# JunyiPeng00/wespeaker_hubert

Hardware: AMD Instinct MI355X
Metric: embeddings/sec on 5s 16kHz utts (higher is better)
Workload: dtype f32 (bf16x3 split MFMA, fp32 accumulate)

## Files before the change

### wespeaker_hubert_amd/csrc/conv_gemm.hip

```cpp
#include "gemm_common.h"

namespace wsp {

namespace {

constexpr int BK = 32;
constexpr int LDK = BK + 4;

template <int WM, int WN, int TM, int TN, int AMODE, bool UNI>
__global__ __launch_bounds__(256, 2) void conv_gemm_f32(const ConvGemmArgs p) {
  constexpr int BM = WM * TM * 32;
  constexpr int BN = WN * TN * 32;
  constexpr int AR = BM / 32;
  constexpr int BR = BN / 32;
  static_assert(WM * WN == 4, "4 waves");

  extern __shared__ __attribute__((aligned(16))) float smem[];
  float* As = smem;
  float* Bs = smem + 2 * BM * LDK;

  const int tid = threadIdx.x;
  const int lane = tid & 63;
  const int wave = tid >> 6;
  const int ntiles = p.N / BN;
// ... 79 lines not shown
}

template <int WM, int WN, int TM, int TN, int AMODE, bool UNI>
void launch_k(const ConvGemmArgs& p, hipStream_t s) {
  constexpr int BM = WM * TM * 32, BN = WN * TN * 32;
  const int nwg = ((p.M + BM - 1) / BM) * (p.N / BN);
  const size_t lds = (size_t)2 * (BM + BN) * LDK * sizeof(float);
  hipLaunchKernelGGL((conv_gemm_f32<WM, WN, TM, TN, AMODE, UNI>), dim3(nwg), dim3(256), lds, s, p);
  WSP_HIP(hipGetLastError());
}

template <int WM, int WN, int TM, int TN>
void launch_tile(const ConvGemmArgs& p, hipStream_t s) {
  const bool uni = uniform_ktiles(p);
  if (p.amode == kAAdd) {
    if (uni) launch_k<WM, WN, TM, TN, kAAdd, true>(p, s);
    else launch_k<WM, WN, TM, TN, kAAdd, false>(p, s);
  } else {
    if (uni) launch_k<WM, WN, TM, TN, kACat, true>(p, s);
    else launch_k<WM, WN, TM, TN, kACat, false>(p, s);
  }
}

}

int conv_gemm_tile_for(int N) { return (N % 128 == 0) ? 0 : 1; }

void launch_conv_gemm(const ConvGemmArgs& args, hipStream_t s) {
  const ConvGemmArgs p = normalized(args);
  check_conv_args(p, "conv_gemm");
  WSP_CHECK(!p.colsum, "conv_gemm: column sums are a bf16x3-kernel epilogue");
  WSP_CHECK(!p.conv2d && p.N % 64 == 0, "conv_gemm (f32): 1-D convs with N % 64 == 0 only");
  WSP_CHECK(!p.gcols || p.gcols % 64 == 0, "conv_gemm (f32): grouped columns must be a multiple of 64");
  WSP_CHECK(!p.sc2d && !p.lnmode, "conv_gemm (f32): conv3 + shortcut and the LayerNorm fold run on tile family 7");
  if (conv_gemm_tile_for(p.N) == 0 && !p.gcols)
    launch_tile<2, 2, 2, 2>(p, s);
  else
    launch_tile<4, 1, 1, 2>(p, s);
}

}
```

### wespeaker_hubert_amd/csrc/conv_gemm_x3.hip

```cpp
#include "conv_gemm_x3_impl.h"

namespace wsp {

int conv_gemm_x3_block_rows(const ConvGemmArgs& p, int variant) {
  if (p.N % 64 != 0 || (p.gcols && p.gcols % 64 != 0)) return 128;
  if (p.gcols || p.N % 128 != 0) return 128;
  return variant == 3 ? 128 : 256;
}

namespace {
__global__ __launch_bounds__(256) void colsum_mean_kernel(const double* __restrict__ part, int bm, int T, int N,
                                                          float* __restrict__ out, int ldo) {
  const int b = blockIdx.y;
  const int n = blockIdx.x * 256 + threadIdx.x;
  if (n >= N) return;
  const long r0 = (long)b * T, r1 = r0 + T;
  double v = 0.0;
  for (long mt = r0 / bm; mt * bm < r1; ++mt) {
    const int slot = (mt * bm) / T == b ? 0 : 1;
    v += part[((size_t)mt * 2 + slot) * N + n];
  }
  out[(long)b * ldo + n] = (float)(v / (double)T);
}
}

void launch_colsum_mean(const double* part, int block_rows, int T, int B, int N, float* out, int ldo,
                        hipStream_t s) {
  WSP_CHECK(block_rows > 0 && T >= block_rows && B > 0 && N > 0, "colsum_mean: bad shape");
  hipLaunchKernelGGL(colsum_mean_kernel, dim3((N + 255) / 256, B), dim3(256), 0, s, part, block_rows, T, N, out,
                     ldo);
  WSP_HIP(hipGetLastError());
}

void launch_conv_gemm_x3(const ConvGemmArgs& args, const void* whi, const void* wlo, int variant,
                         hipStream_t s) {
  const ConvGemmArgs p = normalized(args);
  check_conv_args(p, "conv_gemm_x3");
  if (p.colsum) {
    const int bm = conv_gemm_x3_block_rows(p, variant);
    WSP_CHECK(!p.seg && !p.row_bias && !p.conv2d && p.T >= bm,
              "conv_gemm_x3: column sums need a uniform batch with T >= block rows and no row bias");
  }
  WSP_CHECK(p.Kp % 64 == 0, "conv_gemm_x3: packed K must be a multiple of 64");
  WSP_CHECK(variant >= 3 && variant <= 7, "conv_gemm_x3: tile family must be 3, 4, 5, 6 or 7");
  const __bf16* h = static_cast<const __bf16*>(whi);
  const __bf16* l = static_cast<const __bf16*>(wlo);
  x3::TileFn f;
  WSP_CHECK(!p.lnmode || (variant == 7 && x3::g256_supported(p)),
            "conv_gemm_x3: the LayerNorm fold runs on tile family 7 only");
  WSP_CHECK(!p.sc2d || (variant == 7 && x3::g256_supported(p)),
            "conv_gemm_x3: conv3 + shortcut runs on tile family 7 only (N % 256 == 0, 16-B aligned operands)");
  if (variant == 7 && x3::g256_supported(p)) {
    x3::t_g256(p, h, l, s);
    return;
  }
  if (variant == 7) variant = 6;
  if (p.N % 64 != 0 || (p.gcols && p.gcols % 64 != 0)) {
    f = x3::t_4x1_1x1;
  } else if (p.gcols) {
    f = variant >= 5 ? x3::t_8x1_1x2_sw : x3::t_4x1_1x2;
  } else if (p.N % 128 != 0) {
    f = x3::t_4x1_1x2;
  } else if (variant == 3) {
    f = x3::t_2x2_2x2_sw;
  } else if (variant == 4) {
    f = x3::t_4x2_2x2_sw;
  } else if (p.N % 256 == 0) {
    f = variant == 6 ? x3::t_4x2_2x4_mf16 : x3::t_4x2_2x4_sw1;
  } else {
    f = x3::t_4x2_2x2_sw;
  }
  f(p, h, l, s);
}

}
```

### wespeaker_hubert_amd/csrc/conv_gemm_x3_impl.h

```cpp
#pragma once

#include <type_traits>

#include "gemm_common.h"

namespace wsp {

namespace {

typedef __bf16 bf16x8 __attribute__((ext_vector_type(8)));
typedef __bf16 bf16x4 __attribute__((ext_vector_type(4)));

constexpr int BK = 32;

template <bool SWZ, int MF = 32>
struct Lds {
  static constexpr int ROWB = SWZ ? 64 : 80;
  static constexpr int SKEW = SWZ ? 0 : 64;
  __device__ __forceinline__ static int off(int row, int byte) {
    static_assert(MF == 32 || SWZ, "16x16 fragments need the swizzled rows");
    if constexpr (SWZ && MF == 16)
      return row * 64 + ((((byte >> 4) ^ (0x1320 >> (4 * ((row >> 2) & 3)))) & 3) << 4) + (byte & 15);
    else if constexpr (SWZ) return row * 64 + ((((byte >> 4) ^ (row >> 2)) & 3) << 4) + (byte & 15);
    else return row * 80 + byte;
// ... 269 lines not shown
  if (MF == 32 && p.amode == kAAdd) {
    if constexpr (MF == 32) {
      if (uni)
        launch_x3_k<WM, WN, TM, TN, kAAdd, true, 0, false, SWZ, NSET, MF>(p, whi, wlo, s);
      else
        launch_x3_k<WM, WN, TM, TN, kAAdd, false, 0, false, SWZ, NSET, MF>(p, whi, wlo, s);
    }
  } else if (!uni) {
    launch_x3_k<WM, WN, TM, TN, kACat, false, 0, false, SWZ, NSET, MF>(p, whi, wlo, s);
  } else if (p.role == 1) {
    launch_x3_k<WM, WN, TM, TN, kACat, true, 1, false, SWZ, NSET, MF>(p, whi, wlo, s);
  } else if constexpr (NSET == 2 && TM * TN <= 4) {
    if (p.res && p.role == 2)
      launch_x3_k<WM, WN, TM, TN, kACat, true, 2, false, SWZ, NSET>(p, whi, wlo, s);
    else
      launch_x3_k<WM, WN, TM, TN, kACat, true, 0, false, SWZ, NSET>(p, whi, wlo, s);
  } else {
    launch_x3_k<WM, WN, TM, TN, kACat, true, 0, false, SWZ, NSET, MF>(p, whi, wlo, s);
  }
}

}

namespace x3 {
using TileFn = void (*)(const ConvGemmArgs&, const __bf16*, const __bf16*, hipStream_t);
void t_4x1_1x1(const ConvGemmArgs&, const __bf16*, const __bf16*, hipStream_t);
void t_4x1_1x2(const ConvGemmArgs&, const __bf16*, const __bf16*, hipStream_t);
void t_8x1_1x2_sw(const ConvGemmArgs&, const __bf16*, const __bf16*, hipStream_t);
void t_2x2_2x2_sw(const ConvGemmArgs&, const __bf16*, const __bf16*, hipStream_t);
void t_4x2_2x2_sw(const ConvGemmArgs&, const __bf16*, const __bf16*, hipStream_t);
void t_4x2_2x4_sw1(const ConvGemmArgs&, const __bf16*, const __bf16*, hipStream_t);
void t_4x2_2x4_mf16(const ConvGemmArgs&, const __bf16*, const __bf16*, hipStream_t);
bool g256_supported(const ConvGemmArgs&);
void t_g256(const ConvGemmArgs&, const __bf16*, const __bf16*, hipStream_t);
}

}
```

### wespeaker_hubert_amd/csrc/conv_gemm_x3_t6.hip

```cpp
#include "conv_gemm_x3_impl.h"

namespace wsp {
namespace {

typedef __attribute__((address_space(3))) void lds_void;
constexpr int kGA = 256 * 128, kGW = 256 * 64, kGStage = kGA + 2 * kGW;

__device__ __forceinline__ int g_aslot(int r, int c) { return r * 128 + ((c ^ ((r >> 1) & 5)) << 4); }

__device__ __forceinline__ void g_dma(__amdgpu_buffer_rsrc_t r, unsigned char* lds, int voff) {
  __builtin_amdgcn_raw_ptr_buffer_load_lds(r, (lds_void*)lds, 16, voff, 0, 0, 0);
}

constexpr int kGEpiLd = 132;
constexpr int kGEpiBytes = 8 * 32 * kGEpiLd * 4;
typedef unsigned u32x4 __attribute__((ext_vector_type(4)));

constexpr int kLnMaxParts = 8;
__device__ __forceinline__ void g_ln_row(const ConvGemmArgs& p, int row, float& mu, float& rstd) {
  const float* s = p.ln_in + (size_t)row * p.ln_parts * 2;
  float m = s[0], m2 = s[1];
#pragma unroll
  for (int k = 1; k < kLnMaxParts; ++k) {
    if (k < p.ln_parts) {
// ... 188 lines not shown
      v0 += __shfl_xor(v0, 32);
      double v1 = c1 + __shfl_xor(c1, 16);
      v1 += __shfl_xor(v1, 32);
      rs[4 * pp + jj][0] = v0;
      rs[4 * pp + jj][1] = v1;
      __builtin_amdgcn_sched_barrier(0);
    }
    asm volatile("s_waitcnt lgkmcnt(0)" ::: "memory");
  }
  __syncthreads();
  constexpr int BN = 256;
  double* red = reinterpret_cast<double*>(smem);
  if (lane < 16) {
#pragma unroll
    for (int j = 0; j < 8; ++j)
#pragma unroll
      for (int u = 0; u < 2; ++u) red[(wm * 2 + u) * BN + (wn * 8 + j) * 16 + lane] = rs[j][u];
  }
  __syncthreads();
  const int tid = threadIdx.x;
  if (tid < 2 * BN) {
    const int u = tid / BN, c = tid - u * BN;
    double v = 0.0;
#pragma unroll
    for (int w = 0; w < 4; ++w) v += red[(w * 2 + u) * BN + c];
    p.colsum[((size_t)(m0 / 256) * 2 + u) * p.N + n0 + c] = v;
  }
}

template <int AM, bool CSK, int LNM = 0, int XP = 0>
__global__ __launch_bounds__(512, 1) void conv_gemm_g(const ConvGemmArgs p, const __bf16* __restrict__ whi,
                                                      const __bf16* __restrict__ wlo) {
  using L = Lds<true, 16>;
  constexpr bool DENSE = AM == 1 || AM == 3;
  extern __shared__ __attribute__((aligned(16))) unsigned char smem[];
  const int tid = threadIdx.x;
  const int lane = tid & 63;
  const int wave = tid >> 6;
  const int ntiles = p.N / 256;
  const int mtiles = (p.M + 255) / 256;
  const int wg = xcd_remap(blockIdx.x, ntiles * mtiles);
  const int mt = wg / ntiles;
  const int nt = wg - mt * ntiles;
  const int m0 = mt * 256;
  const int n0 = nt * 256;

  const int ac0 = 4 * ((lane & 7) ^ ((lane >> 4) & 1)), ac1 = ac0 ^ 16;
  int a_r[4], a_t[DENSE ? 1 : 4], a_l[DENSE ? 1 : 4], a_s[AM == 3 ? 4 : 1];
#pragma unroll
  for (int i = 0; i < 4; ++i) {
    const int m = m0 + (4 * wave + i) * 8 + (lane >> 3);
    if constexpr (DENSE) {
      a_r[i] = m < p.M ? m : -1;
      if constexpr (AM == 3) {
        const int fto = p.Fo * p.To;
        const int b = m / fto, fo = (m - b * fto) / p.To, to = m - b * fto - fo * p.To;
        a_s[i] = m < p.M ? (b * p.Fi + fo * p.stride) * p.Ti + to * p.stride : -1;
      }
    } else if (p.seg) {
      const int mm = m < p.M ? m : p.M - 1;
      const int b = seg_of(p.seg, p.nseg, mm);
      const int t = (mm - p.seg[b]) * p.stride;
      const int* is = p.iseg ? p.iseg : p.seg;
      a_r[i] = is[b] + t;
      a_t[i] = (m < p.M) ? t : -0x40000000;
      a_l[i] = is[b + 1] - is[b];
    } else {
// ... 42 lines not shown
        const int offk = tap * p.dil - p.pad;
        const int tt = a_t[i] + offk;
        const bool ok = k < p.K && tt >= 0 && tt < a_l[i];
        g_dma(ra, st + (4 * wave + i) * 1024, ok ? ((a_r[i] + offk) * ld + k - tap * p.cin) * 4 : kOOB);
      } else {
        const int tt = a_t[i] + off;
        const bool ok = tt >= 0 && tt < a_l[i];
        g_dma(ra, st + (4 * wave + i) * 1024, ok ? ((a_r[i] + off) * ld + cl + (i & 1 ? ac1 : ac0)) * 4 : kOOB);
      }
    }
#pragma unroll
    for (int i = 0; i < 2; ++i) {
      if (!(part & 2)) break;
      const int o = woff[i] + kt * 64;
      g_dma(rwh, st + kGA + (2 * wave + i) * 1024, o);
      g_dma(rwl, st + kGA + kGW + (2 * wave + i) * 1024, o);
    }
    if (!(part & 2)) return;
    ct += 32;
    if (ct >= p.cin) {
      ct -= p.cin;
      ++jt;
    }
  };

  const int wm = wave >> 1, wn = wave & 1;
  const int r16 = lane & 15, qk = lane >> 4;
  f32x4 acc[4][8];
#pragma unroll
  for (int i = 0; i < 4; ++i)
#pragma unroll
    for (int j = 0; j < 8; ++j) acc[i][j] = f32x4{0.f, 0.f, 0.f, 0.f};
  bf16x8 ah[2], al[2], bh[4], bl[4];
  auto rdA = [&](const unsigned char* st, int ih) {
#pragma unroll
    for (int i = 0; i < 2; ++i) {
      const int r = wm * 64 + (ih * 2 + i) * 16 + r16;
      const f32x4 x0 = *reinterpret_cast<const f32x4*>(st + g_aslot(r, 2 * qk));
      const f32x4 x1 = *reinterpret_cast<const f32x4*>(st + g_aslot(r, 2 * qk + 1));
      if constexpr (XP == 1 || XP == 4) {
        ah[i] = __builtin_bit_cast(bf16x8, x0);
        al[i] = __builtin_bit_cast(bf16x8, x1);
        continue;
      }
#pragma unroll
      for (int e = 0; e < 4; ++e) {
        const __bf16 h0 = (__bf16)x0[e], h1 = (__bf16)x1[e];
        ah[i][e] = h0;
        ah[i][4 + e] = h1;
        al[i][e] = (__bf16)(x0[e] - (float)h0);
        al[i][4 + e] = (__bf16)(x1[e] - (float)h1);
      }
    }
  };
  auto rdB = [&](const unsigned char* st, int jh) {
#pragma unroll
    for (int j = 0; j < 4; ++j) {
      const int o = L::off(wn * 128 + (jh * 4 + j) * 16 + r16, qk * 16);
      bh[j] = *reinterpret_cast<const bf16x8*>(st + kGA + o);
      bl[j] = *reinterpret_cast<const bf16x8*>(st + kGA + kGW + o);
    }
  };
  auto mm = [&](int ih, int jh) {
#pragma unroll
    for (int i = 0; i < 2; ++i)
#pragma unroll
      for (int j = 0; j < 4; ++j) {
        f32x4& c = acc[ih * 2 + i][jh * 4 + j];
        c = __builtin_amdgcn_mfma_f32_16x16x32_bf16(al[i], bh[j], c, 0, 0, 0);
        c = __builtin_amdgcn_mfma_f32_16x16x32_bf16(ah[i], bl[j], c, 0, 0, 0);
        c = __builtin_amdgcn_mfma_f32_16x16x32_bf16(ah[i], bh[j], c, 0, 0, 0);
      }
  };

  float lmu = 0.f, lrs = 1.f;
  if constexpr ((LNM & 6) != 0) g_ln_row(p, min(m0 + wm * 64 + lane, p.M - 1), lmu, lrs);
  dma(0, 0);
  dma(1, 1);
  asm volatile("s_waitcnt vmcnt(8)" ::: "memory");
  __builtin_amdgcn_s_barrier();
  for (int kt = 0; kt < nk; ++kt) {
    const int buf = kt & 1;
    const unsigned char* st = smem + buf * kGStage;
    if constexpr (XP == 2) {
      rdA(st, 0);
      rdB(st, 0);
      mm(0, 0);
      __builtin_amdgcn_sched_barrier(0);
      if (kt >= 1 && kt + 1 < nk) dma(kt + 1, buf ^ 1, 1);
      __builtin_amdgcn_sched_barrier(0);
      rdB(st, 1);
      mm(0, 1);
      __builtin_amdgcn_sched_barrier(0);
      if (kt >= 1 && kt + 1 < nk) dma(kt + 1, buf ^ 1, 2);
      __builtin_amdgcn_sched_barrier(0);
      rdA(st, 1);
      mm(1, 1);
      rdB(st, 0);
      mm(1, 0);
      asm volatile("s_waitcnt vmcnt(0) lgkmcnt(0)" ::: "memory");
      __builtin_amdgcn_s_barrier();
      __builtin_amdgcn_sched_barrier(0);
      continue;
    }
    rdA(st, 0);
    rdB(st, 0);
    mm(0, 0);
    rdB(st, 1);
    mm(0, 1);
    rdA(st, 1);
    mm(1, 1);
    rdB(st, 0);
    mm(1, 0);
    if constexpr (XP >= 3) {
      asm volatile("s_waitcnt lgkmcnt(0)" ::: "memory");
      continue;
    }
    asm volatile("s_waitcnt vmcnt(0) lgkmcnt(0)" ::: "memory");
    __builtin_amdgcn_s_barrier();
    __builtin_amdgcn_sched_barrier(0);
    if (kt + 2 < nk) dma(kt + 2, buf);
  }
#define WSP_GEPI(RB, RES)                                                                                   \
  switch (p.act) {                                                                                         \
    case kActRelu: g_epilogue_rows<kActRelu, RB, RES>(p, acc, m0, n0, wm, wn, wave, lane, smem); break;    \
    case kActTanh: g_epilogue_rows<kActTanh, RB, RES>(p, acc, m0, n0, wm, wn, wave, lane, smem); break;    \
    case kActGelu: g_epilogue_rows<kActGelu, RB, RES>(p, acc, m0, n0, wm, wn, wave, lane, smem); break;    \
    default: g_epilogue_rows<kActNone, RB, RES>(p, acc, m0, n0, wm, wn, wave, lane, smem); break;          \
  }
  if constexpr (LNM != 0) {
    if constexpr ((LNM & 5) != 0)
      g_epilogue_rows<kActNone, false, true, LNM>(p, acc, m0, n0, wm, wn, wave, lane, smem, lmu, lrs);
    else if (p.act == kActGelu)
      g_epilogue_rows<kActGelu, false, false, LNM>(p, acc, m0, n0, wm, wn, wave, lane, smem, lmu, lrs);
    else
      g_epilogue_rows<kActNone, false, false, LNM>(p, acc, m0, n0, wm, wn, wave, lane, smem, lmu, lrs);
  } else if constexpr (CSK) {
    switch (p.act) {
      case kActRelu: g_epilogue_cs<kActRelu>(p, acc, m0, n0, wm, wn, wave, lane, smem); break;
      case kActTanh: g_epilogue_cs<kActTanh>(p, acc, m0, n0, wm, wn, wave, lane, smem); break;
      case kActGelu: g_epilogue_cs<kActGelu>(p, acc, m0, n0, wm, wn, wave, lane, smem); break;
      default: g_epilogue_cs<kActNone>(p, acc, m0, n0, wm, wn, wave, lane, smem); break;
    }
  } else if (p.res) {
    WSP_GEPI(false, true)
  } else if (p.row_bias) {
    WSP_GEPI(true, false)
  } else {
    WSP_GEPI(false, false)
  }
#undef WSP_GEPI
}

#ifdef WSP_G7_XP
constexpr int kBStages = 4;
// ... 160 lines not shown
    default: g_epilogue_rows<kActNone, RB, RES>(p, acc, m0, n0, wm, wn, wave, lane, smem); break;          \
  }
  if constexpr (CSK) {
    switch (p.act) {
      case kActRelu: g_epilogue_cs<kActRelu>(p, acc, m0, n0, wm, wn, wave, lane, smem); break;
      case kActTanh: g_epilogue_cs<kActTanh>(p, acc, m0, n0, wm, wn, wave, lane, smem); break;
      case kActGelu: g_epilogue_cs<kActGelu>(p, acc, m0, n0, wm, wn, wave, lane, smem); break;
      default: g_epilogue_cs<kActNone>(p, acc, m0, n0, wm, wn, wave, lane, smem); break;
    }
  } else if (p.res) {
    WSP_GBEPI(false, true)
  } else if (p.row_bias) {
    WSP_GBEPI(true, false)
  } else {
    WSP_GBEPI(false, false)
  }
#undef WSP_GBEPI
}
#endif

}

namespace x3 {

bool g256_supported(const ConvGemmArgs& p) {
  auto a16 = [](const void* q) { return (reinterpret_cast<uintptr_t>(q) & 15) == 0; };
  const bool aligned = a16(p.out) && p.ldo % 4 == 0 && a16(p.bias) && a16(p.scale) && a16(p.shift) &&
                       a16(p.row_bias) && a16(p.res) && (!p.res || p.ldres % 4 == 0);
  return aligned && p.N % 256 == 0 && !p.conv2d && !p.gcols && p.amode == kACat &&
         (uniform_ktiles(p) || (p.cseg[1] >= p.cin && !p.colsum)) &&
         (!p.sc2d || (uniform_ktiles(p) && !p.colsum && !p.lnmode && !p.row_bias));
}

void t_g256(const ConvGemmArgs& p, const __bf16* h, const __bf16* l, hipStream_t s) {
  const int nwg = ((p.M + 255) / 256) * (p.N / 256);
  constexpr int lds0 = 2 * kGStage > kGEpiBytes ? 2 * kGStage : kGEpiBytes;
  constexpr int lds = lds0 > kGCsBytes ? lds0 : kGCsBytes;
  const bool dense = p.taps == 1 && p.pad == 0 && p.stride == 1 && !p.iseg && (p.seg || p.Ti == p.T);
  const int am = !uniform_ktiles(p) ? 2 : dense ? 1 : 0;
  if (p.sc2d) {
    hipLaunchKernelGGL((conv_gemm_g<3, false>), dim3(nwg), dim3(512), lds, s, p, h, l);
    WSP_HIP(hipGetLastError());
    return;
  }
  if (p.lnmode) {
    WSP_CHECK(am == 1 && !p.colsum && !p.row_bias && !p.scale && p.N % 128 == 0 &&
                  ((p.lnmode & 1) == 0 || (p.ln_out && p.res && p.act == kActNone)) &&
                  ((p.lnmode & 6) == 0 || (p.ln_in && p.ln_parts >= 1 && p.ln_parts <= kLnMaxParts)) && ((p.lnmode & 2) == 0 || (p.ln_cs && !p.res)) &&
                  (p.lnmode != 2 || p.act == kActNone || p.act == kActGelu) &&
                  ((p.lnmode & 4) == 0 || (p.ln_g && p.ln_b && p.res && p.act == kActNone)),
              "conv_gemm_x3: LayerNorm fold needs a dense 1x1 GEMM and its operands (fold: no activation or GELU)");
    switch (p.lnmode) {
      case 1: hipLaunchKernelGGL((conv_gemm_g<1, false, 1>), dim3(nwg), dim3(512), lds, s, p, h, l); break;
      case 2: hipLaunchKernelGGL((conv_gemm_g<1, false, 2>), dim3(nwg), dim3(512), lds, s, p, h, l); break;
      case 4: hipLaunchKernelGGL((conv_gemm_g<1, false, 4>), dim3(nwg), dim3(512), lds, s, p, h, l); break;
      case 5: hipLaunchKernelGGL((conv_gemm_g<1, false, 5>), dim3(nwg), dim3(512), lds, s, p, h, l); break;
      default: WSP_CHECK(false, "conv_gemm_x3: lnmode must be 1, 2, 4 or 5");
    }
    WSP_HIP(hipGetLastError());
    return;
  }
  if (p.colsum && am == 1)
    hipLaunchKernelGGL((conv_gemm_g<1, true>), dim3(nwg), dim3(512), lds, s, p, h, l);
  else if (p.colsum && am == 0)
    hipLaunchKernelGGL((conv_gemm_g<0, true>), dim3(nwg), dim3(512), lds, s, p, h, l);
  else if (am == 1)
    hipLaunchKernelGGL((conv_gemm_g<1, false>), dim3(nwg), dim3(512), lds, s, p, h, l);
  else if (am == 0)
    hipLaunchKernelGGL((conv_gemm_g<0, false>), dim3(nwg), dim3(512), lds, s, p, h, l);
  else
    hipLaunchKernelGGL((conv_gemm_g<2, false>), dim3(nwg), dim3(512), lds, s, p, h, l);
  WSP_HIP(hipGetLastError());
// ... 53 lines not shown
```

### wespeaker_hubert_amd/csrc/ecapa_model.cpp

```cpp
#include "model_impl.h"

namespace wsp {

void Model::Impl::build_ecapa_params() {
  const int64_t C = this->C, w = C / 8;
  add("layer1.conv.weight", {C, feat_dim, 5});
  add("layer1.conv.bias", {C});
  add_bn("layer1.bn", C);
  for (int li = 2; li <= 4; ++li) {
    const std::string p = "layer" + std::to_string(li) + ".se_res2block";
    add(p + ".0.conv.weight", {C, C, 1});
    add(p + ".0.conv.bias", {C});
    add_bn(p + ".0.bn", C);
    for (int i = 0; i < 7; ++i) {
      add(p + ".1.convs." + std::to_string(i) + ".weight", {w, w, 3});
      add(p + ".1.convs." + std::to_string(i) + ".bias", {w});
    }
    for (int i = 0; i < 7; ++i) add_bn(p + ".1.bns." + std::to_string(i), w);
    add(p + ".2.conv.weight", {C, C, 1});
    add(p + ".2.conv.bias", {C});
    add_bn(p + ".2.bn", C);
    add(p + ".3.linear1.weight", {128, C});
    add(p + ".3.linear1.bias", {128});
    add(p + ".3.linear2.weight", {C, 128});
// ... 111 lines not shown
  w.h1 = c.take(M * C);
  w.h2 = c.take(M * C);
  w.h3 = c.take(M * C);
  w.gmean = c.take(B * C);
  w.ghid = c.take(B * 128);
  w.gate = c.take(B * C);
  w.xp = c.take(M * 1536);
  w.att = c.take(M * 128);
  w.logit = c.take(M * 1536);
  w.gstats = c.take(B * 3072);
  w.rowb = c.take(B * 128);
  w.pooled = c.take(B * 3072);
  w.sesum = reinterpret_cast<double*>(c.take(((M + 127) / 128) * 2 * C * 2));
  w.floats = c.off;
  return w;
}
}

size_t Model::Impl::ecapa_ws_floats(int B, size_t M) const { return ecapa_ws(C, B, M, nullptr).floats; }

void Model::Impl::forward_ecapa(const float* feats, int B, int T, float* embed, float* ws, hipStream_t s,
                                const int* seg, int M_seg) {
  const int M = seg ? M_seg : B * T, w = C / 8;
  const EcapaWs W = ecapa_ws(C, B, M, ws);
  float* const* x = W.x;
  float *h1 = W.h1, *h2 = W.h2, *h3 = W.h3, *xp = W.xp;
  const int se_bm = precision == 1 ? conv_gemm_x3_block_rows(ConvGemmArgs{.N = C}, x3_variant) : 0;
  const bool se_fused = precision == 1 && !seg && T >= se_bm;
  auto gemm3 = [&](const char* tag, ConvGemmArgs& g, const ConvW& cw, int dil, int pad, float* out, int ldo) {
    g.lda[0] = g.lda[1] = g.lda[2] = C;
    fill(g, cw, M, T, dil, pad, out, ldo, kActRelu, nullptr, true, seg, B);
    run(tag, 2.0 * M * cw.N * cw.K, s, [&] { launch(g, cw, s); });
  };

  gemm("layer1", layer1, feats, feat_dim, x[1], C, M, T, 1, 2, kActRelu, s, seg, B);
  for (int li = 0; li < 3; ++li) {
    const Block& b = blk[li];
    const int dil = li + 2;
    const float* xin = x[li + 1];
    gemm("conv1x1_CxC", b.c1, xin, C, h1, C, M, T, 1, 0, kActRelu, s, seg, B, nullptr, true, 1);
    if (precision == 1 && res2_fused && b.r2w) {
      Res2Args r{};
      r.x = h1;
      r.out = h2;
      r.ldx = r.ldo = C;
      r.M = M;
      r.T = T;
      r.dil = dil;
      r.variant = w == 128 ? res2_variant : std::min(res2_variant, 3);
      r.rout = res2_chain_rout(dil, r.variant, M);
      r.seg = seg;
      r.nseg = B;
      r.w = b.r2w;
      r.bias = b.r2b;
      r.scale = b.r2s;
      r.shift = b.r2t;
      run("res2_k3", 7 * 2.0 * M * w * 3 * w, s, [&] { launch_res2_chain(r, w, s); });
    } else {
      for (int i = 0; i < 7; ++i) {
        ConvGemmArgs g{};
        g.amode = i == 0 ? kACat : kAAdd;
        if (i == 0) {
          one_operand(g, h1, C, w);
        } else {
          g.a[0] = h1 + i * w;
          g.a[1] = h2 + (i - 1) * w;
          g.a[2] = h1;
        }
        gemm3("res2_k3", g, b.res2[i], dil, dil, h2 + i * w, C);
      }
    }
    {
      ConvGemmArgs g{};
      g.amode = kACat;
      g.a[0] = h2;
      g.a[1] = h1 + 7 * w;
      g.a[2] = h1;
      g.cseg[1] = 7 * w;
      g.cseg[2] = g.cseg[3] = C;
      g.role = 1;
      if (se_fused) g.colsum = W.sesum;
      gemm3("conv1x1_CxC", g, b.c3, 1, 0, h3, C);
    }
    run("se", 0, s, [&] {
      if (se_fused) launch_colsum_mean(W.sesum, se_bm, T, B, C, W.gmean, C, s);
      else launch_frame_stats(h3, C, B, T, C, W.gmean, C, 0, 0, s, seg);
      launch_small_linear({W.gmean, C, b.se1.wt, b.se1.bias, W.ghid, 128, B, C, 128, 1}, s);
      launch_small_linear({W.ghid, 128, b.se2.wt, b.se2.bias, W.gate, C, B, 128, C, 3}, s);
      launch_residual_scale(cat_gate && li == 2 ? nullptr : xin, h3, W.gate, x[li + 2], B, T, C, s, seg, M);
    });
  }
  {
    ConvGemmArgs g{};
    g.amode = kACat;
    g.a[0] = x[2];
    g.a[1] = x[3];
    g.a[2] = x[4];
    g.cseg[1] = C;
    g.cseg[2] = 2 * C;
    g.cseg[3] = 3 * C;
    gemm3("conv_cat", g, cat_gate ? conv_g : conv, 1, 0, xp, 1536);
  }
  if (glob) {
    run("glob_ctx", 0, s, [&] {
      launch_frame_stats(xp, 1536, B, T, 1536, W.gstats, 3072, 1, 1536, s, seg);
      launch_small_linear({W.gstats, 3072, pool1_ctx.wt, pool1_ctx.bias, W.rowb, 128, B, 3072, 128, 0}, s);
    });
  }
  gemm("pool_linear1", pool1, xp, 1536, W.att, 128, M, T, 1, 0, kActTanh, s, seg, B, glob ? W.rowb : nullptr, !glob);
  if (precision == 1 && astp_fused_on) {
    AstpArgs a{W.att, xp, 1536, B, T, 1536, seg, pool2_frag, pool2.bias, 1e-7f, W.pooled};
    run("astp", 2.0 * M * 1536 * 128, s, [&] { launch_astp_fused(a, s); });
  } else {
    gemm("pool_linear2", pool2, W.att, 128, W.logit, 1536, M, T, 1, 0, kActNone, s, seg, B);
    run("astp", 0, s, [&] { launch_astp_pool(W.logit, xp, B, T, 1536, W.pooled, s, seg); });
  }
  run("head", 0, s, [&] {
    launch_small_linear({W.pooled, 3072, head.wt, head.bias, embed, embed_dim, B, 3072, embed_dim, 0}, s);
  });
}

}
```

### wespeaker_hubert_amd/csrc/kernels.h

```cpp
#pragma once

#include <vector>

#include "common.h"

namespace wsp {

enum AMode { kACat = 0, kAAdd = 1 };
enum Act { kActNone = 0, kActRelu = 1, kActTanh = 2, kActGelu = 3 };

struct ConvGemmArgs {
  const float* a[3];
  int lda[3];
  int cseg[4];
  int cin, taps, dil, pad;
  int M, T, N;
  const float* w;
  int K, Kp;
  const float* bias;
  const float* row_bias;
  const float* res;
  int ldres;
  const float* scale;
  const float* shift;
  float* out;
  int ldo;
  int act;
  int amode;
  int role;
  int conv2d;
  int Fi, Ti, Fo, To, stride, kw;
  int sc2d;
  int gcols, gcin;
  const int* seg;
  const int* iseg;
  int nseg;
  double* colsum;
  int lnmode;
  float* ln_out;
  const float* ln_in;
  int ln_parts;
  const float* ln_cs;
  const float* ln_g;
  const float* ln_b;
  float ln_eps;
};

inline ConvGemmArgs normalized(ConvGemmArgs p) {
  if (!p.conv2d && !p.sc2d) {
    if (p.stride <= 0) p.stride = 1;
    if (p.Ti <= 0) p.Ti = p.T;
  }
  return p;
}

int conv_gemm_x3_block_rows(const ConvGemmArgs& p, int variant);
void launch_colsum_mean(const double* part, int block_rows, int T, int B, int N, float* out, int ldo,
                        hipStream_t s);
void launch_conv_gemm_x3(const ConvGemmArgs& p, const void* whi, const void* wlo, int variant,
                         hipStream_t s);


void launch_conv_gemm(const ConvGemmArgs& p, hipStream_t s);
int conv_gemm_tile_for(int N);

struct SmallLinearArgs {
  const float* in;
  int ldin;
  const float* wt;
  const float* bias;
  float* out;
  int ldo;
  int R, K, N;
  int act;
  float* scratch = nullptr;
  size_t scratch_floats = 0;
};
void launch_small_linear(const SmallLinearArgs& p, hipStream_t s);
size_t small_linear_scratch_floats(int R, int N, int K);


void launch_frame_stats(const float* x, int ldx, int B, int T, int C, float* out, int ldo,
                        int with_std, int std_off, hipStream_t s, const int* seg = nullptr);

void launch_residual_scale(const float* x, const float* h, const float* g, float* out, int B,
                           int T, int C, hipStream_t s, const int* seg = nullptr, int M = 0);

void launch_astp_pool(const float* e, const float* x, int B, int T, int C, float* out,
                      hipStream_t s, const int* seg = nullptr, float var_floor = 1e-7f);

int simam_chunks(int B, int rows);
void launch_simam(const float* z, const float* res, float* out, int B, int rows, int C, double* part, float* coef,
                  hipStream_t s);
// ... 76 lines not shown
```

### wespeaker_hubert_amd/csrc/model.cpp

```cpp
#include "model_impl.h"

namespace wsp {

int detail::chunk_for(int B, size_t bytes) {
  const int bc = std::min((int)std::max<size_t>(1, kOperandCap / bytes), B);
  const int chunks = (B + bc - 1) / bc;
  return (B + chunks - 1) / chunks;
}

void Model::Impl::add(const std::string& n, std::vector<int64_t> shape) {
  idx[n] = (int)params.size();
  params.push_back(Param{n, std::move(shape), {}, false});
}
void Model::Impl::add_bn(const std::string& p, int64_t c) {
  add(p + ".weight", {c});
  add(p + ".bias", {c});
  add(p + ".running_mean", {c});
  add(p + ".running_var", {c});
  add(p + ".num_batches_tracked", {});
}
const std::vector<float>& Model::Impl::P(const std::string& n) const {
  auto it = idx.find(n);
  WSP_CHECK(it != idx.end(), "missing parameter " + n);
  const Param& p = params[it->second];
// ... 292 lines not shown
  WSP_CHECK(m.finalized, "forward before finalize");
  WSP_CHECK(seg != nullptr && B > 0 && M >= B, "segmented batch needs offsets, B >= 1 and M >= B rows");
  WSP_CHECK((size_t)M * 1536 < (1u << 31) / 4, "segmented batch too large");
  WSP_CHECK(ws_bytes >= workspace_bytes_segments(B, M), "workspace too small");
  float* wsf = reinterpret_cast<float*>((reinterpret_cast<uintptr_t>(ws) + 255) & ~uintptr_t(255));
  m.forward_ecapa(feats, B, 1, embed, wsf, s, seg, M);
}

void Model::profile(bool on) {
  if (on && !impl->prof)
    for (auto& kv : impl->prof_map) {
      kv.second.used = 0;
      kv.second.flops = 0;
    }
  impl->prof = on;
}

namespace {
struct Opt {
  const char* key;
  int Model::Impl::*field;
  int lo, hi, hole;
  const char* err;
};
using I = Model::Impl;
constexpr int kNoHole = -1000;
const Opt kOpts[] = {
    {"precision", &I::precision, 0, 1, kNoHole, "precision must be 0 (f32) or 1 (bf16x3)"},
    {"streams", &I::streams, 1, 8, kNoHole, "streams must be 1..8"},
    {"layer", &I::h_layer_sel, -1, 12, kNoHole, "layer must be -1 (weighted sum) or 0..12"},
    {"in_planes", &I::m_ch, 32, 64, kNoHole, "in_planes must be 32 or 64"},
    {"res2_fused", &I::res2_fused, 0, 1, kNoHole, "res2_fused must be 0 or 1"},
    {"cat_gate", &I::cat_gate, 0, 1, kNoHole, "cat_gate must be 0 or 1"},
    {"res_prefetch", &I::res_prefetch, 0, 1, kNoHole, "res_prefetch must be 0 or 1"},
    {"res_tail", &I::res_tail, 0, 2, kNoHole, "res_tail must be 0 (off), 1 (tail + next conv1) or 2 (tail alone)"},
    {"sc_fuse", &I::sc_fuse, 0, 3, kNoHole, "sc_fuse must be 0 .. 3 (bit 0: one GEMM, bit 1: in the tail)"},
    {"c1_stage_fuse", &I::c1_stage_fuse, 0, 1, kNoHole, "c1_stage_fuse must be 0 or 1"},
    {"astp_fused", &I::astp_fused_on, 0, 3, kNoHole,
     "astp_fused must be 0 (linear2 GEMM + pooling kernel) or 1 (fused)"},
    {"attn_pipe", &I::attn_pipe, 0, 1, kNoHole, "attn_pipe must be 0 or 1"},
    {"pos_conv", &I::pos_conv, 0, 1, kNoHole,
     "pos_conv must be 0 (grouped implicit GEMM) or 1 (direct grouped conv)"},
    {"ln_fold", &I::ln_fold, 0, 1, kNoHole, "ln_fold must be 0 (LayerNorm kernels) or 1 (folded into the GEMMs)"},
    {"tail_batch", &I::tail_batch, 0, 1, kNoHole,
     "tail_batch must be 0 (CNN layers 4-6 per chunk) or 1 (batch-wide)"},
    {"res2_variant", &I::res2_variant, 0, 4, 1,
     "res2_variant must be 0 (4 waves, 2 x 2), 2 (4 waves on N, 4 W k-steps in flight), 3 (8 waves) "
     "or 4 (halo-free strips, c1024 widths; else as 3)"},
    {"x3_variant", &I::x3_variant, 0, 9, kNoHole,
     "x3_variant must be 3, 4, 5, 6 (5 on 16x16x32 MFMAs) or 7 (6 staged by LDS-DMA)"},
    {"conv3x3_img", &I::conv3x3_img_on, 0, 3, kNoHole,
     "conv3x3_img must be 0 (off), 1 (32 / 64 channels) or 2 / 3 (also 128)"},
};
const Opt& find_opt(const std::string& key) {
  for (const Opt& o : kOpts)
    if (key == o.key) return o;
  throw InvalidArg{"unknown option " + key};
}
}

void Model::set_option(const std::string& key, int value) {
  Impl& m = *impl;
  if (key == "attn_lds" || key == "conv1x1_rows") return;
  const Opt& o = find_opt(key);
  if (key == "layer") {
    WSP_CHECK(m.hubert, "option 'layer' applies to the HuBERT front end");
// ... 42 lines not shown
```

### wespeaker_hubert_amd/csrc/model_impl.h

```cpp
#pragma once

#include <hip/hip_runtime.h>

#include <cmath>
#include <cstdint>
#include <algorithm>
#include <map>
#include <string>
#include <vector>

#include "kernels.h"
#include "model.h"
#include "pack.h"
#include "res2_chain.h"
#include "astp_fused.h"
#include "conv3x3_img.h"

namespace wsp {

namespace detail {

constexpr double kBnEps = 1e-5;

struct DevBuf {
// ... 86 lines not shown
};

struct ProfEntry {
  std::vector<std::pair<hipEvent_t, hipEvent_t>> ev;
  size_t used = 0;
  double flops = 0;
};

struct Model::Impl {
  std::string arch;
  bool ecapa = true;
  int C = 512;
  bool glob = false;
  int feat_dim = 80, embed_dim = 192;
  bool emb_bn = false, two_emb = false;
  std::vector<Param> params;
  std::map<std::string, int> idx;
  bool finalized = false;
  int device = 0;
  DevBuf dev;

  ConvW layer1;
  struct Block {
    ConvW c1, c3, res2[7];
    LinW se1, se2;
    void* r2w = nullptr;
    float *r2b = nullptr, *r2s = nullptr, *r2t = nullptr;
  } blk[3];
  int res2_fused = 1;
  int res2_variant = 4;
  ConvW conv, pool1, pool2;
  ConvW conv_g;
  int cat_gate = 1;
  void* pool2_frag = nullptr;
  int astp_fused_on = 1;
  LinW pool1_ctx;
  LinW head;
  void build_ecapa_params();
  void pack_res2(Block& b, const std::string& p, int w);
  void finalize_ecapa();
  int ecapa_chunk(int B, int T) const;
  size_t ecapa_ws_floats(int B, size_t M) const;
  void forward_ecapa(const float* feats, int B, int T, float* embed, float* ws, hipStream_t s,
                     const int* seg = nullptr, int M_seg = 0);

  bool bottleneck = true;
  int nblocks[4] = {0, 0, 0, 0};
  int m_ch = 32;
  float* stem_w = nullptr;
  float* stem_b = nullptr;
  int conv3x3_img_on = 2;
  int res_prefetch = 1;
  int res_tail = 1;
  int sc_fuse = 3;
  int c1_stage_fuse = 1;
  bool img_ok(const ConvW& cw, int C) const { return cw.frag && conv3x3_img_on && (C <= 64 || conv3x3_img_on >= 2); }
  struct RBlock {
    ConvW c1, c2, c3, sc;
    ConvW c3sc;
    void* w3acc = nullptr;
    void* w3scx = nullptr;
    float* b3scx = nullptr;
    void* w1frag = nullptr;
    bool has_sc = false;
    int stride = 1, in_planes = 0, planes = 0, out_planes = 0;
    std::string name;
// ... 123 lines not shown
```

Before: 25620.

## Fold last SE gate scaling into the concatenated conv GEMM A-operand load

Adds a gated A-tail instance of the tile-family-7 bf16x3 GEMM. It stages per-utterance SE gate vectors in LDS and multiplies the last concatenated input segment by them as A tiles are read. For the third ECAPA block, the separate residual-scale kernel is skipped and conv_cat reads the unscaled h3 directly. This removes one elementwise pass over an activation tensor, at the cost of extra LDS and a per-element multiply inside the GEMM's inner loop, and only applies when the dense and uniform-batch shape conditions hold.

```diff
diff --git a/wespeaker_hubert_amd/csrc/conv_gemm.hip b/wespeaker_hubert_amd/csrc/conv_gemm.hip
--- a/wespeaker_hubert_amd/csrc/conv_gemm.hip
+++ b/wespeaker_hubert_amd/csrc/conv_gemm.hip
@@ -135,7 +135,8 @@
   WSP_CHECK(!p.colsum, "conv_gemm: column sums are a bf16x3-kernel epilogue");
   WSP_CHECK(!p.conv2d && p.N % 64 == 0, "conv_gemm (f32): 1-D convs with N % 64 == 0 only");
   WSP_CHECK(!p.gcols || p.gcols % 64 == 0, "conv_gemm (f32): grouped columns must be a multiple of 64");
-  WSP_CHECK(!p.sc2d && !p.lnmode, "conv_gemm (f32): conv3 + shortcut and the LayerNorm fold run on tile family 7");
+  WSP_CHECK(!p.sc2d && !p.lnmode && !p.gate,
+            "conv_gemm (f32): conv3 + shortcut, the LayerNorm fold and the gated A tail run on tile family 7");
   if (conv_gemm_tile_for(p.N) == 0 && !p.gcols)
     launch_tile<2, 2, 2, 2>(p, s);
   else
diff --git a/wespeaker_hubert_amd/csrc/conv_gemm_x3.hip b/wespeaker_hubert_amd/csrc/conv_gemm_x3.hip
--- a/wespeaker_hubert_amd/csrc/conv_gemm_x3.hip
+++ b/wespeaker_hubert_amd/csrc/conv_gemm_x3.hip
@@ -32,6 +32,10 @@
   WSP_HIP(hipGetLastError());
 }
 
+bool conv_gemm_x3_gate_ok(const ConvGemmArgs& args, int variant) {
+  return variant == 7 && args.gate && x3::g256_gate_supported(normalized(args));
+}
+
 void launch_conv_gemm_x3(const ConvGemmArgs& args, const void* whi, const void* wlo, int variant,
                          hipStream_t s) {
   const ConvGemmArgs p = normalized(args);
@@ -50,6 +54,8 @@
             "conv_gemm_x3: the LayerNorm fold runs on tile family 7 only");
   WSP_CHECK(!p.sc2d || (variant == 7 && x3::g256_supported(p)),
             "conv_gemm_x3: conv3 + shortcut runs on tile family 7 only (N % 256 == 0, 16-B aligned operands)");
+  WSP_CHECK(!p.gate || (variant == 7 && x3::g256_gate_supported(p)),
+            "conv_gemm_x3: the gated A tail runs on tile family 7 only (conv_gemm_x3_gate_ok)");
   if (variant == 7 && x3::g256_supported(p)) {
     x3::t_g256(p, h, l, s);
     return;
diff --git a/wespeaker_hubert_amd/csrc/conv_gemm_x3_impl.h b/wespeaker_hubert_amd/csrc/conv_gemm_x3_impl.h
--- a/wespeaker_hubert_amd/csrc/conv_gemm_x3_impl.h
+++ b/wespeaker_hubert_amd/csrc/conv_gemm_x3_impl.h
@@ -325,6 +325,7 @@
 void t_4x2_2x4_sw1(const ConvGemmArgs&, const __bf16*, const __bf16*, hipStream_t);
 void t_4x2_2x4_mf16(const ConvGemmArgs&, const __bf16*, const __bf16*, hipStream_t);
 bool g256_supported(const ConvGemmArgs&);
+bool g256_gate_supported(const ConvGemmArgs&);
 void t_g256(const ConvGemmArgs&, const __bf16*, const __bf16*, hipStream_t);
 }
 
diff --git a/wespeaker_hubert_amd/csrc/conv_gemm_x3_t6.hip b/wespeaker_hubert_amd/csrc/conv_gemm_x3_t6.hip
--- a/wespeaker_hubert_amd/csrc/conv_gemm_x3_t6.hip
+++ b/wespeaker_hubert_amd/csrc/conv_gemm_x3_t6.hip
@@ -244,7 +244,9 @@
 __global__ __launch_bounds__(512, 1) void conv_gemm_g(const ConvGemmArgs p, const __bf16* __restrict__ whi,
                                                       const __bf16* __restrict__ wlo) {
   using L = Lds<true, 16>;
-  constexpr bool DENSE = AM == 1 || AM == 3;
+  constexpr bool DENSE = AM == 1 || AM == 3 || AM == 4;
+  constexpr bool GATE = AM == 4;
+  static_assert(!GATE || (!CSK && LNM == 0 && XP == 0), "the gated instance: plain epilogues only");
   extern __shared__ __attribute__((aligned(16))) unsigned char smem[];
   const int tid = threadIdx.x;
   const int lane = tid & 63;
@@ -353,12 +355,20 @@
 #pragma unroll
     for (int j = 0; j < 8; ++j) acc[i][j] = f32x4{0.f, 0.f, 0.f, 0.f};
   bf16x8 ah[2], al[2], bh[4], bl[4];
-  auto rdA = [&](const unsigned char* st, int ih) {
+  const int g_nb = GATE ? min((m0 / p.T + 1) * p.T, p.M) - m0 : 0;
+  const int g_slot = GATE ? (p.K - p.gate_k0) * 4 : 0;
+  auto rdA = [&](auto gated, const unsigned char* st, int ih, const unsigned char* gp = nullptr) {
+#pragma clang fp contract(off)
 #pragma unroll
     for (int i = 0; i < 2; ++i) {
       const int r = wm * 64 + (ih * 2 + i) * 16 + r16;
-      const f32x4 x0 = *reinterpret_cast<const f32x4*>(st + g_aslot(r, 2 * qk));
-      const f32x4 x1 = *reinterpret_cast<const f32x4*>(st + g_aslot(r, 2 * qk + 1));
+      f32x4 x0 = *reinterpret_cast<const f32x4*>(st + g_aslot(r, 2 * qk));
+      f32x4 x1 = *reinterpret_cast<const f32x4*>(st + g_aslot(r, 2 * qk + 1));
+      if constexpr (decltype(gated)::value) {
+        const unsigned char* gr = gp + (r >= g_nb ? g_slot : 0);
+        x0 = x0 * *reinterpret_cast<const f32x4*>(gr);
+        x1 = x1 * *reinterpret_cast<const f32x4*>(gr + 16);
+      }
       if constexpr (XP == 1 || XP == 4) {
         ah[i] = __builtin_bit_cast(bf16x8, x0);
         al[i] = __builtin_bit_cast(bf16x8, x1);
@@ -396,15 +406,29 @@
 
   float lmu = 0.f, lrs = 1.f;
   if constexpr ((LNM & 6) != 0) g_ln_row(p, min(m0 + wm * 64 + lane, p.M - 1), lmu, lrs);
+  if constexpr (GATE) {
+    const int ppu = g_slot >> 10, b0 = m0 / p.T;
+    const __amdgpu_buffer_rsrc_t rg = make_rsrc(p.gate);
+#pragma unroll
+    for (int i = 0; i < 4; ++i) {
+      const int q = 8 * i + wave;
+      if (q >= 2 * ppu) break;
+      const int u = q >= ppu ? 1 : 0;
+      const bool ok = (b0 + u) * p.T < p.M;
+      g_dma(rg, smem + 2 * kGStage + q * 1024, ok ? ((b0 + u) * p.ldg + (q - u * ppu) * 256 + lane * 4) * 4 : kOOB);
+    }
+  }
   dma(0, 0);
   dma(1, 1);
   asm volatile("s_waitcnt vmcnt(8)" ::: "memory");
   __builtin_amdgcn_s_barrier();
-  for (int kt = 0; kt < nk; ++kt) {
+  auto ktile = [&](auto gated, int kt) {
     const int buf = kt & 1;
     const unsigned char* st = smem + buf * kGStage;
+    const unsigned char* gp =
+        decltype(gated)::value ? smem + 2 * kGStage + (kt * BK - p.gate_k0 + 8 * qk) * 4 : nullptr;
     if constexpr (XP == 2) {
-      rdA(st, 0);
+      rdA(gated, st, 0);
       rdB(st, 0);
       mm(0, 0);
       __builtin_amdgcn_sched_barrier(0);
@@ -415,33 +439,37 @@
       __builtin_amdgcn_sched_barrier(0);
       if (kt >= 1 && kt + 1 < nk) dma(kt + 1, buf ^ 1, 2);
       __builtin_amdgcn_sched_barrier(0);
-      rdA(st, 1);
+      rdA(gated, st, 1);
       mm(1, 1);
       rdB(st, 0);
       mm(1, 0);
       asm volatile("s_waitcnt vmcnt(0) lgkmcnt(0)" ::: "memory");
       __builtin_amdgcn_s_barrier();
       __builtin_amdgcn_sched_barrier(0);
-      continue;
-    }
-    rdA(st, 0);
+      return;
+    }
+    rdA(gated, st, 0, gp);
     rdB(st, 0);
     mm(0, 0);
     rdB(st, 1);
     mm(0, 1);
-    rdA(st, 1);
+    rdA(gated, st, 1, gp);
     mm(1, 1);
     rdB(st, 0);
     mm(1, 0);
     if constexpr (XP >= 3) {
       asm volatile("s_waitcnt lgkmcnt(0)" ::: "memory");
-      continue;
+      return;
     }
     asm volatile("s_waitcnt vmcnt(0) lgkmcnt(0)" ::: "memory");
     __builtin_amdgcn_s_barrier();
     __builtin_amdgcn_sched_barrier(0);
     if (kt + 2 < nk) dma(kt + 2, buf);
-  }
+  };
+  const int ktg = GATE ? p.gate_k0 / BK : nk;
+  for (int kt = 0; kt < ktg; ++kt) ktile(std::false_type{}, kt);
+  if constexpr (GATE)
+    for (int kt = ktg; kt < nk; ++kt) ktile(std::true_type{}, kt);
 #define WSP_GEPI(RB, RES)                                                                                   \
   switch (p.act) {                                                                                         \
     case kActRelu: g_epilogue_rows<kActRelu, RB, RES>(p, acc, m0, n0, wm, wn, wave, lane, smem); break;    \
@@ -668,12 +696,29 @@
          (!p.sc2d || (uniform_ktiles(p) && !p.colsum && !p.lnmode && !p.row_bias));
 }
 
+bool g256_gate_supported(const ConvGemmArgs& p) {
+  if (!p.gate || !g256_supported(p) || !uniform_ktiles(p)) return false;
+  const bool dense = p.taps == 1 && p.pad == 0 && p.stride == 1 && !p.iseg && !p.seg && p.Ti == p.T;
+  const int gk = p.K - p.gate_k0;
+  return dense && p.T >= 256 && p.M % p.T == 0 && !p.colsum && !p.lnmode && !p.sc2d && p.K == p.Kp &&
+         p.gate_k0 >= 0 && p.gate_k0 % 32 == 0 && gk > 0 && gk % 128 == 0 && gk <= 4096 && p.ldg >= gk &&
+         p.ldg % 4 == 0 && (reinterpret_cast<uintptr_t>(p.gate) & 15) == 0 &&
+         (long long)(p.M / p.T) * p.ldg * 4 < (long long)kOOB;
+}
+
 void t_g256(const ConvGemmArgs& p, const __bf16* h, const __bf16* l, hipStream_t s) {
   const int nwg = ((p.M + 255) / 256) * (p.N / 256);
   constexpr int lds0 = 2 * kGStage > kGEpiBytes ? 2 * kGStage : kGEpiBytes;
   constexpr int lds = lds0 > kGCsBytes ? lds0 : kGCsBytes;
   const bool dense = p.taps == 1 && p.pad == 0 && p.stride == 1 && !p.iseg && (p.seg || p.Ti == p.T);
   const int am = !uniform_ktiles(p) ? 2 : dense ? 1 : 0;
+  if (p.gate) {
+    WSP_CHECK(g256_gate_supported(p), "conv_gemm_x3: the gated A tail needs a dense 1x1 GEMM over a uniform batch");
+    const int ldsg = std::max(lds, 2 * kGStage + 2 * (p.K - p.gate_k0) * 4);
+    hipLaunchKernelGGL((conv_gemm_g<4, false>), dim3(nwg), dim3(512), ldsg, s, p, h, l);
+    WSP_HIP(hipGetLastError());
+    return;
+  }
   if (p.sc2d) {
     hipLaunchKernelGGL((conv_gemm_g<3, false>), dim3(nwg), dim3(512), lds, s, p, h, l);
     WSP_HIP(hipGetLastError());
diff --git a/wespeaker_hubert_amd/csrc/ecapa_model.cpp b/wespeaker_hubert_amd/csrc/ecapa_model.cpp
--- a/wespeaker_hubert_amd/csrc/ecapa_model.cpp
+++ b/wespeaker_hubert_amd/csrc/ecapa_model.cpp
@@ -167,6 +167,28 @@
     fill(g, cw, M, T, dil, pad, out, ldo, kActRelu, nullptr, true, seg, B);
     run(tag, 2.0 * M * cw.N * cw.K, s, [&] { launch(g, cw, s); });
   };
+
+  ConvGemmArgs gcat{};
+  gcat.amode = kACat;
+  gcat.a[0] = x[2];
+  gcat.a[1] = x[3];
+  gcat.a[2] = x[4];
+  gcat.cseg[1] = C;
+  gcat.cseg[2] = 2 * C;
+  gcat.cseg[3] = 3 * C;
+  gcat.lda[0] = gcat.lda[1] = gcat.lda[2] = C;
+  const ConvW& wcat = cat_gate ? conv_g : conv;
+  bool fold = false;
+  if (cat_gate && gate_fold && precision == 1) {
+    ConvGemmArgs g = gcat;
+    g.a[2] = h3;
+    g.gate = W.gate;
+    g.ldg = C;
+    g.gate_k0 = 2 * C;
+    fill(g, wcat, M, T, 1, 0, xp, 1536, kActRelu, nullptr, true, seg, B);
+    fold = conv_gemm_x3_gate_ok(g, x3_variant);
+    if (fold) gcat = g;
+  }
 
   gemm("layer1", layer1, feats, feat_dim, x[1], C, M, T, 1, 2, kActRelu, s, seg, B);
   for (int li = 0; li < 3; ++li) {
@@ -222,20 +244,13 @@
       else launch_frame_stats(h3, C, B, T, C, W.gmean, C, 0, 0, s, seg);
       launch_small_linear({W.gmean, C, b.se1.wt, b.se1.bias, W.ghid, 128, B, C, 128, 1}, s);
       launch_small_linear({W.ghid, 128, b.se2.wt, b.se2.bias, W.gate, C, B, 128, C, 3}, s);
+    });
+    if (li == 2 && fold) continue;
+    run("se.scale", 0, s, [&] {
       launch_residual_scale(cat_gate && li == 2 ? nullptr : xin, h3, W.gate, x[li + 2], B, T, C, s, seg, M);
     });
   }
-  {
-    ConvGemmArgs g{};
-    g.amode = kACat;
-    g.a[0] = x[2];
-    g.a[1] = x[3];
-    g.a[2] = x[4];
-    g.cseg[1] = C;
-    g.cseg[2] = 2 * C;
-    g.cseg[3] = 3 * C;
-    gemm3("conv_cat", g, cat_gate ? conv_g : conv, 1, 0, xp, 1536);
-  }
+  gemm3("conv_cat", gcat, wcat, 1, 0, xp, 1536);
   if (glob) {
     run("glob_ctx", 0, s, [&] {
       launch_frame_stats(xp, 1536, B, T, 1536, W.gstats, 3072, 1, 1536, s, seg);
diff --git a/wespeaker_hubert_amd/csrc/kernels.h b/wespeaker_hubert_amd/csrc/kernels.h
--- a/wespeaker_hubert_amd/csrc/kernels.h
+++ b/wespeaker_hubert_amd/csrc/kernels.h
@@ -44,6 +44,8 @@
   const float* ln_g;
   const float* ln_b;
   float ln_eps;
+  const float* gate;
+  int ldg, gate_k0;
 };
 
 inline ConvGemmArgs normalized(ConvGemmArgs p) {
@@ -59,6 +61,7 @@
                         hipStream_t s);
 void launch_conv_gemm_x3(const ConvGemmArgs& p, const void* whi, const void* wlo, int variant,
                          hipStream_t s);
+bool conv_gemm_x3_gate_ok(const ConvGemmArgs& p, int variant);
 
 
 void launch_conv_gemm(const ConvGemmArgs& p, hipStream_t s);
diff --git a/wespeaker_hubert_amd/csrc/model.cpp b/wespeaker_hubert_amd/csrc/model.cpp
--- a/wespeaker_hubert_amd/csrc/model.cpp
+++ b/wespeaker_hubert_amd/csrc/model.cpp
@@ -348,6 +348,7 @@
     {"in_planes", &I::m_ch, 32, 64, kNoHole, "in_planes must be 32 or 64"},
     {"res2_fused", &I::res2_fused, 0, 1, kNoHole, "res2_fused must be 0 or 1"},
     {"cat_gate", &I::cat_gate, 0, 1, kNoHole, "cat_gate must be 0 or 1"},
+    {"gate_fold", &I::gate_fold, 0, 1, kNoHole, "gate_fold must be 0 or 1"},
     {"res_prefetch", &I::res_prefetch, 0, 1, kNoHole, "res_prefetch must be 0 or 1"},
     {"res_tail", &I::res_tail, 0, 2, kNoHole, "res_tail must be 0 (off), 1 (tail + next conv1) or 2 (tail alone)"},
     {"sc_fuse", &I::sc_fuse, 0, 3, kNoHole, "sc_fuse must be 0 .. 3 (bit 0: one GEMM, bit 1: in the tail)"},
diff --git a/wespeaker_hubert_amd/csrc/model_impl.h b/wespeaker_hubert_amd/csrc/model_impl.h
--- a/wespeaker_hubert_amd/csrc/model_impl.h
+++ b/wespeaker_hubert_amd/csrc/model_impl.h
@@ -142,6 +142,7 @@
   ConvW conv, pool1, pool2;
   ConvW conv_g;
   int cat_gate = 1;
+  int gate_fold = 1;
   void* pool2_frag = nullptr;
   int astp_fused_on = 1;
   LinW pool1_ctx;
```

Result: faster. 25900 (median of 6 runs) (+1.1%).
